# MiniMax-AI/VTP

Hardware: AMD Instinct MI355X
Metric: images/sec/node VTP-B f16d64 256x256 train step (higher is better)
Workload: dtype bf16

## Files before the change

vtp_amd/csrc/attention_resident.hip:

```cpp
#include "common.h"
#include <algorithm>
#include <cstdio>
#include <cstdlib>
#include "vtp_hip.h"

namespace vtp {

constexpr float LOG2E_R = 1.4426950408889634f;
constexpr float LN2_R = 0.6931471805599453f;
constexpr int RES_MAXN = 320;
constexpr int RES_SPLIT_COLS = 4;

struct AttnResArgs {
  const bf16 *q, *k, *v, *o, *d_o;
  bf16 *out, *dq, *dk, *dv;
  float* lse;
  float* delta;
  const bf16 *rope_sin, *rope_cos;
  int rope_prefix;
  int B, N, heads, npad;
  long sb, sn, sbo, sno;
  float scale;
  int stagger;
  long long* timing;
};

#define BWD_STAMP(i)                                                                                                     \
  do {                                                                                                                   \
    if (__builtin_expect(p.timing != nullptr, 0) && lane == 0)                                                           \
      p.timing[((((size_t)blockIdx.z * gridDim.y + blockIdx.y) * gridDim.x + blockIdx.x) * 16 + wave) * 4 + (i)] = wall_clock64(); \
  } while (0)

__device__ __forceinline__ int swz_key(int r) { return (((r >> 1) & 1) << 2) | ((r >> 2) & 3); }

__device__ __forceinline__ void stage_resident(const bf16* __restrict__ base, long sn, int N, int npad, char* lds, int wave,
                                               int nwaves, int lane) {
  const int rr = lane >> 3, cp = lane & 7;
  for (int piece = wave; piece < (npad >> 3); piece += nwaves) {
    const int row = piece * 8 + rr;
    const int c = cp ^ swz_key(row);
    const bf16* src = base + (long)min(row, N - 1) * sn + c * 8;
    __builtin_amdgcn_global_load_lds((const __attribute__((address_space(1))) void*)src,
                                     (__attribute__((address_space(3))) void*)(lds + piece * 1024), 16, 0, 0);
  }
}

__device__ __forceinline__ bf16x8 frag_row(const char* lds, int row0, int ks, int lane) {
  const int r = row0 + (lane & 31);
  return *(const bf16x8*)(lds + r * 128 + (((2 * ks + (lane >> 5)) ^ swz_key(r)) << 4));
}
__device__ __forceinline__ bf16x8 frag_tr(const char* lds, int dblk, int row0, int ks, int lane) {
  const int i = lane & 15, g = (lane >> 4) & 1, hi = lane >> 5;
  const int r = row0 + ks * 16 + hi * 4 + (i >> 2);
  const int col = dblk * 32 + g * 16 + (i & 3) * 4;
  const char* p0 = lds + r * 128 + (((col >> 3) ^ swz_key(r)) << 4) + ((col & 7) << 1);
  const char* p1 = lds + (r + 8) * 128 + (((col >> 3) ^ swz_key(r + 8)) << 4) + ((col & 7) << 1);
  bf16x4 lo = __builtin_amdgcn_ds_read_tr16_b64_v4bf16((__attribute__((address_space(3))) bf16x4*)p0);
  bf16x4 hi4 = __builtin_amdgcn_ds_read_tr16_b64_v4bf16((__attribute__((address_space(3))) bf16x4*)p1);
  return __builtin_shufflevector(lo, hi4, 0, 1, 2, 3, 4, 5, 6, 7);
}

__device__ __forceinline__ int row_part(int lane) {
  const int r = lane & 31;
  return r * 128 + (((lane >> 5) ^ swz_key(r)) << 4);
}
__device__ __forceinline__ int tr_part(int lane, int half) {
  const int i = lane & 15, g = (lane >> 4) & 1, hi = lane >> 5;
  const int r = hi * 4 + (i >> 2) + 8 * half;
  const int col = g * 16 + (i & 3) * 4;
  return r * 128 + (((col >> 3) ^ swz_key(r)) << 4) + ((col & 7) << 1);
}
__device__ __forceinline__ int lds_addr(int lane_part, int uniform_part) {
  int a;
// ... 123 lines not shown
  for (int kb = 0; kb < nkb; ++kb) {
    f32x16 s;
    zero16r(s);
#pragma unroll
    for (int ks = 0; ks < 4; ++ks) s = __builtin_amdgcn_mfma_f32_32x32x16_bf16(frag_row(Ks, kb * 32, ks, lane), qf[ks], s, 0, 0, 0);
#pragma unroll
    for (int r = 0; r < 16; ++r) s[r] = fast_exp2(s[r] * sc2 - m2);
    if (kb == last) {
#pragma unroll
      for (int r = 0; r < 16; ++r)
        if (kb * 32 + (r & 3) + 8 * (r >> 2) + 4 * hi >= p.N) s[r] = 0.f;
    }
#pragma unroll
    for (int r = 0; r < 16; ++r) l += s[r];
    const bf16x8 pf0 = pack8r(s, 0), pf1 = pack8r(s, 8);
#pragma unroll
    for (int db = 0; db < 2; ++db) {
      oacc[db] = __builtin_amdgcn_mfma_f32_32x32x16_bf16(frag_tr(Vs, db, kb * 32, 0, lane), pf0, oacc[db], 0, 0, 0);
      oacc[db] = __builtin_amdgcn_mfma_f32_32x32x16_bf16(frag_tr(Vs, db, kb * 32, 1, lane), pf1, oacc[db], 0, 0, 0);
    }
  }
  l += __shfl_xor(l, 32, 64);
  if (qi >= p.N) return;
  const float inv = 1.f / l;
  bf16* orow = p.out + (long)b * p.sbo + (long)qi * p.sno + h * 64;
#pragma unroll
  for (int db = 0; db < 2; ++db)
#pragma unroll
    for (int g = 0; g < 4; ++g) {
      f32x4 v;
#pragma unroll
      for (int e = 0; e < 4; ++e) v[e] = oacc[db][4 * g + e] * inv;
      *(bf16x4*)(orow + db * 32 + 8 * g + 4 * hi) = __builtin_convertvector(v, bf16x4);
    }
  if (hi == 0 && p.lse) p.lse[((long)b * p.heads + h) * p.N + qi] = (m2 + log2f(l)) * LN2_R;
}

__device__ __forceinline__ float both_halves_sum(float x) {
  const auto r = __builtin_amdgcn_permlane32_swap(__float_as_uint(x), __float_as_uint(x), false, false);
  return __uint_as_float(r[0]) + __uint_as_float(r[1]);
}

__device__ __forceinline__ float max3f(float a, float b, float c) {
  float r;
  asm("v_max3_f32 %0, %1, %2, %3" : "=v"(r) : "v"(a), "v"(b), "v"(c));
  return r;
}
__device__ __forceinline__ float max2f(float a, float b) {
  float r;
  asm("v_max_f32 %0, %1, %2" : "=v"(r) : "v"(a), "v"(b));
  return r;
}

constexpr float LAZY_LOG2 = 6.f;

template <int T>
__device__ __forceinline__ void attn_key_loop(const char* Ks, const char* Vs, const bf16x8 (&qf)[T][4], int N, int nkb, int kb0, int step,
                                              float sc2, int lane, f32x16 (&oacc)[T][2], float (&m)[T], float (&l)[T],
                                              int stream_ops = 0) {
  const int hi = lane >> 5, last = nkb - 1;
  const f32x16 zero = {0.f, 0.f, 0.f, 0.f, 0.f, 0.f, 0.f, 0.f, 0.f, 0.f, 0.f, 0.f, 0.f, 0.f, 0.f, 0.f};
  const f32x2 sc2v = {sc2, sc2};
#pragma unroll
  for (int t = 0; t < T; ++t) {
    oacc[t][0] = zero;
    oacc[t][1] = zero;
    m[t] = -INFINITY;
    l[t] = 0.f;
  }
  for (int kb = kb0; kb < nkb; kb += step) {
    if (stream_ops > 0 && (kb == 2 || kb == 5)) {
      wait_vmcnt_upto(__builtin_amdgcn_readfirstlane(kb == 2 ? stream_ops * max(nkb - 5, 0) : 0));
      __builtin_amdgcn_s_barrier();
      asm volatile("" ::: "memory");
    }
    f32x16 s[T];
    {
      bf16x8 kf[4];
#pragma unroll
      for (int ks = 0; ks < 4; ++ks) kf[ks] = frag_row(Ks, kb * 32, ks, lane);
#pragma unroll
      for (int t = 0; t < T; ++t) {
        s[t] = __builtin_amdgcn_mfma_f32_32x32x16_bf16(kf[0], qf[t][0], zero, 0, 0, 0);
#pragma unroll
        for (int ks = 1; ks < 4; ++ks) s[t] = __builtin_amdgcn_mfma_f32_32x32x16_bf16(kf[ks], qf[t][ks], s[t], 0, 0, 0);
      }
    }
    bf16x8 vf[2][2];
#pragma unroll
    for (int db = 0; db < 2; ++db)
#pragma unroll
      for (int ks = 0; ks < 2; ++ks) vf[db][ks] = frag_tr(Vs, db, kb * 32, ks, lane);
    if (kb == last && (N & 31)) {
#pragma unroll
      for (int t = 0; t < T; ++t)
#pragma unroll
        for (int r = 0; r < 16; ++r)
          if (kb * 32 + (r & 3) + 8 * (r >> 2) + 4 * hi >= N) s[t][r] = -INFINITY;
    }
    float mn[T];
    bool moved = false;
#pragma unroll
    for (int t = 0; t < T; ++t) {
      float bm = max3f(s[t][0], s[t][1], s[t][2]);
#pragma unroll
      for (int r = 3; r < 15; r += 2) bm = max3f(bm, s[t][r], s[t][r + 1]);
// ... 48 lines not shown
  for (int db = 0; db < 2; ++db)
#pragma unroll
    for (int j = 0; j < 2; ++j) {
      uint32_t x[2], y[2];
#pragma unroll
      for (int w = 0; w < 2; ++w) {
        const f32x2 vx = {o[db][8 * j + 2 * w] * inv, o[db][8 * j + 2 * w + 1] * inv};
        const f32x2 vy = {o[db][8 * j + 4 + 2 * w] * inv, o[db][8 * j + 4 + 2 * w + 1] * inv};
        const bf16x2 bx = __builtin_convertvector(vx, bf16x2), by = __builtin_convertvector(vy, bf16x2);
        x[w] = __builtin_bit_cast(uint32_t, bx);
        y[w] = __builtin_bit_cast(uint32_t, by);
      }
      uint32_t out[4];
#pragma unroll
      for (int w = 0; w < 2; ++w) {
        const auto r = __builtin_amdgcn_permlane32_swap(x[w], y[w], false, false);
        out[w] = r[0];
        out[2 + w] = r[1];
      }
      if (valid) {
        typedef __attribute__((ext_vector_type(4))) uint32_t u32x4;
        *(u32x4*)(orow + db * 32 + 16 * j + 8 * hi) = u32x4{out[0], out[1], out[2], out[3]};
      }
    }
}

__device__ __forceinline__ void stage_piece_asm(const bf16* base, long sn, int N, int piece, unsigned img_off, int lane) {
  const int row = piece * 8 + (lane >> 3);
  const int c = (lane & 7) ^ swz_key(row);
  const unsigned voff = (unsigned)(min(row, N - 1) * (int)sn + c * 8) * 2u;
  const unsigned dst = __builtin_amdgcn_readfirstlane(img_off + piece * 1024);
  unsigned keep;
  asm volatile("s_mov_b32 %0, m0\n\ts_mov_b32 m0, %3\n\ts_nop 0\n\tglobal_load_lds_dwordx4 %1, %2\n\ts_mov_b32 m0, %0"
               : "=&s"(keep)
               : "v"(voff), "s"(base), "s"(dst)
               : "memory");
}
__device__ __forceinline__ void stage_block_asm(const bf16* kbase, const bf16* vbase, long sn, int N, int kb, unsigned img, int wave,
                                                int nwaves, int lane) {
  for (int j = wave; j < 4; j += nwaves) {
    stage_piece_asm(kbase, sn, N, kb * 4 + j, 0, lane);
    stage_piece_asm(vbase, sn, N, kb * 4 + j, img, lane);
  }
}

#define ATTN_TSTAMP(i)                                                                            \
  do {                                                                                            \
    if (p.delta && blockIdx.x == 3 && blockIdx.y == 5 && lane == 0)                               \
      ((long long*)p.delta)[wave * 8 + (i)] = __builtin_readcyclecounter();                       \
  } while (0)

__global__ __launch_bounds__(256, 2) void attn_fwd_res2_kernel(const AttnResArgs p) {
  extern __shared__ __attribute__((aligned(16))) char smem[];
  char* Ks = smem;
  char* Vs = smem + p.npad * 128;
  float* part = (float*)(smem + 2 * p.npad * 128);
  const int lane = threadIdx.x & 63, wave = threadIdx.x >> 6, nwaves = blockDim.x >> 6, hi = lane >> 5;
  const int h = blockIdx.x, b = blockIdx.y;
  const bf16* qb = p.q + (long)b * p.sb + h * 64;
  const int ntiles = p.npad >> 5, nkb = ntiles, q0 = wave * 64;
  ATTN_TSTAMP(0);
  const bool split_last = (ntiles & 1) && ntiles > 1;
  const int qL = (ntiles - 1) * 32;
  bf16x8 qf[2][4], qfl[1][4];
#pragma unroll
  for (int t = 0; t < 2; ++t) {
    const bf16* qr = qb + (long)min(q0 + 32 * t + (lane & 31), p.N - 1) * p.sn + hi * 8;
#pragma unroll
    for (int ks = 0; ks < 4; ++ks) qf[t][ks] = *(const bf16x8*)(qr + ks * 16);
  }
  if (split_last) {
    const bf16* qr = qb + (long)min(qL + (lane & 31), p.N - 1) * p.sn + hi * 8;
#pragma unroll
    for (int ks = 0; ks < 4; ++ks) qfl[0][ks] = *(const bf16x8*)(qr + ks * 16);
  }
  const bf16* kbase = p.k + (long)b * p.sb + h * 64;
  const bf16* vbase = p.v + (long)b * p.sb + h * 64;
  const unsigned img = p.npad * 128;
  stage_block_asm(kbase, vbase, p.sn, p.N, 0, img, wave, nwaves, lane);
  if (nkb > 1) stage_block_asm(kbase, vbase, p.sn, p.N, 1, img, wave, nwaves, lane);
  __builtin_amdgcn_s_waitcnt(0x0F70);
  ATTN_TSTAMP(1);
  __builtin_amdgcn_s_barrier();
  asm volatile("" ::: "memory");
  ATTN_TSTAMP(2);
  for (int kb = 2; kb < nkb; ++kb) stage_block_asm(kbase, vbase, p.sn, p.N, kb, img, wave, nwaves, lane);
  const int stream_ops = 2 * ((4 - wave + nwaves - 1) / nwaves);
  const float sc2 = p.scale * LOG2E_R;
  const long srow0 = ((long)b * p.heads + h) * p.N;
  {
    f32x16 oacc[2][2];
    float m[2], l[2];
    const bool two = q0 + 32 < p.npad && !(split_last && q0 + 32 >= qL);
    if (two) attn_key_loop<2>(Ks, Vs, qf, p.N, nkb, 0, 1, sc2, lane, oacc, m, l, stream_ops);
    else {
      f32x16 (&o1)[1][2] = *(f32x16(*)[1][2])&oacc;
      attn_key_loop<1>(Ks, Vs, *(const bf16x8(*)[1][4])&qf, p.N, nkb, 0, 1, sc2, lane, o1, *(float(*)[1])&m, *(float(*)[1])&l,
                       stream_ops);
    }
    ATTN_TSTAMP(3);
#pragma unroll
    for (int t = 0; t < 2; ++t) {
      if (t == 1 && !two) break;
      const int qi = q0 + 32 * t + (lane & 31);
      const float lt = both_halves_sum(l[t]);
      const bool valid = qi < p.N;
      store_o_row(p.out + (long)b * p.sbo + (long)min(qi, p.N - 1) * p.sno + h * 64, oacc[t], 1.f / lt, hi, valid);
      if (valid && hi == 0 && p.lse) p.lse[srow0 + qi] = (m[t] + log2f(lt)) * LN2_R;
    }
  }
  ATTN_TSTAMP(4);
  if (!split_last) return;
  const int cols = p.N - qL;
  {
    f32x16 oacc[1][2];
    float m[1], l[1];
    attn_key_loop<1>(Ks, Vs, qfl, p.N, nkb, wave, nwaves, sc2, lane, oacc, m, l);
    const float lt = both_halves_sum(l[0]);
    if ((lane & 31) < cols) {
      float* dst = part + ((wave * cols + (lane & 31)) * 2 + hi) * 34;
      dst[0] = m[0];
      dst[1] = lt;
#pragma unroll
      for (int r = 0; r < 16; ++r) {
        dst[2 + r] = oacc[0][0][r];
        dst[18 + r] = oacc[0][1][r];
      }
    }
  }
  ATTN_TSTAMP(5);
  __syncthreads();
  ATTN_TSTAMP(6);
  if (wave != 0) return;
  {
    const int c = min(lane & 31, cols - 1);
    float M = -INFINITY;
    for (int w = 0; w < nwaves; ++w) M = fmaxf(M, part[((w * cols + c) * 2 + hi) * 34]);
    f32x16 o[2];
    zero16r(o[0]);
    zero16r(o[1]);
    float L = 0.f;
    for (int w = 0; w < nwaves; ++w) {
      const float* src = part + ((w * cols + c) * 2 + hi) * 34;
      const float sc = fast_exp2(src[0] - M);
      L += src[1] * sc;
#pragma unroll
      for (int r = 0; r < 16; ++r) {
        o[0][r] += src[2 + r] * sc;
        o[1][r] += src[18 + r] * sc;
      }
    }
    const int qi = qL + (lane & 31);
    const bool valid = (lane & 31) < cols;
    store_o_row(p.out + (long)b * p.sbo + (long)min(qi, p.N - 1) * p.sno + h * 64, o, 1.f / L, hi, valid);
    if (valid && hi == 0 && p.lse) p.lse[srow0 + qi] = (M + log2f(L)) * LN2_R;
  }
}

__global__ __launch_bounds__(640) void attn_bwd_dq_res_kernel(const AttnResArgs p) {
  extern __shared__ __attribute__((aligned(16))) char smem[];
  char* Ks = smem;
  char* Vs = smem + p.npad * 128;
  const int lane = threadIdx.x & 63, wave = threadIdx.x >> 6, nwaves = blockDim.x >> 6, hi = lane >> 5;
  const int h = blockIdx.x, b = blockIdx.y;
// ... 167 lines not shown
      for (int e2 = 0; e2 < 2; ++e2) {
        const int r = 4 * g + 2 * e2;
        f32x2 e = {s[r], s[r + 1]}, gq = {dp[r], dp[r + 1]};
        e = __builtin_elementwise_fma(e, sc2v, f32x2{l4[2 * e2], l4[2 * e2 + 1]});
        gq = __builtin_elementwise_fma(gq, scv, f32x2{d4[2 * e2], d4[2 * e2 + 1]});
        e[0] = fast_exp2(e[0]);
        e[1] = fast_exp2(e[1]);
        if (qblk == last && (p.N & 31)) {
          if (qblk * 32 + 8 * g + 4 * hi + 2 * e2 >= p.N) e[0] = 0.f;
          if (qblk * 32 + 8 * g + 4 * hi + 2 * e2 + 1 >= p.N) e[1] = 0.f;
        }
        pr[r] = e[0];
        pr[r + 1] = e[1];
        e *= gq;
        s[r] = e[0];
        s[r + 1] = e[1];
      }
    }
    const bf16x8 p0 = pack8r(pr, 0), p1 = pack8r(pr, 8), d0 = pack8r(s, 0), d1 = pack8r(s, 8);
#pragma unroll
    for (int db = 0; db < 2; ++db) {
      const int tq0 = lds_addr(tpart[db][0], q_off), tq1 = lds_addr(tpart[db][1], q_off);
      const int tg0 = lds_addr(tpart[db][0], q_off + g_off), tg1 = lds_addr(tpart[db][1], q_off + g_off);
      dv[db] = __builtin_amdgcn_mfma_f32_32x32x16_bf16(frag_tr_at(tg0, tg1, 0), p0, dv[db], 0, 0, 0);
      dv[db] = __builtin_amdgcn_mfma_f32_32x32x16_bf16(frag_tr_at(tg0, tg1, 1), p1, dv[db], 0, 0, 0);
      dk[db] = __builtin_amdgcn_mfma_f32_32x32x16_bf16(frag_tr_at(tq0, tq1, 0), d0, dk[db], 0, 0, 0);
      dk[db] = __builtin_amdgcn_mfma_f32_32x32x16_bf16(frag_tr_at(tq0, tq1, 1), d1, dk[db], 0, 0, 0);
    }
  }
  BWD_STAMP(2);
  if (ki < p.N) {
  bf16* krow = p.dk + (long)b * p.sb + (long)ki * p.sn + h * 64;
  bf16* vrow = p.dv + (long)b * p.sb + (long)ki * p.sn + h * 64;
  const bool rot = p.rope_sin && ki >= p.rope_prefix;
  const long t = (long)(ki - p.rope_prefix) * 64;
#pragma unroll
  for (int g = 0; g < 4; ++g) {
    f32x4 lo, hv, c0, c1;
#pragma unroll
    for (int e = 0; e < 4; ++e) {
      lo[e] = dk[0][4 * g + e];
      hv[e] = dk[1][4 * g + e];
      c0[e] = dv[0][4 * g + e];
      c1[e] = dv[1][4 * g + e];
    }
    store_grad_pair(krow, 8 * g + 4 * hi, lo, hv, rot ? p.rope_sin : nullptr, p.rope_cos, t);
    store_grad_pair(vrow, 8 * g + 4 * hi, c0, c1, nullptr, nullptr, 0);
  }
  }
  BWD_STAMP(3);
}

constexpr int PB_WAVES = 8;
constexpr int PB_XROWS = 2;

__device__ __forceinline__ int stage_image_asm(const bf16* base, long sn, int N, int npad, unsigned img_off, int wave, int nwaves,
                                               int lane) {
  int n = 0;
  for (int piece = wave; piece < (npad >> 3); piece += nwaves, ++n) stage_piece_asm(base, sn, N, piece, img_off, lane);
  return n;
}

__device__ __forceinline__ void dq_step(const bf16x8 (&qf)[4], const bf16x8 (&dof)[4], f32x16 (&dq)[2], const int (&rpart)[4],
                                        const int (&tpart)[2][2], int koff, int img, f32x2 sc2v, f32x2 nlse, f32x2 scv, f32x2 ndlt,
                                        int key0, int N, bool mask, int hi) {
  f32x16 s, dp;
  zero16r(s);
  zero16r(dp);
#pragma unroll
  for (int ks = 0; ks < 4; ++ks) {
    s = __builtin_amdgcn_mfma_f32_32x32x16_bf16(frag_row_at(lds_addr(rpart[ks], koff)), qf[ks], s, 0, 0, 0);
    dp = __builtin_amdgcn_mfma_f32_32x32x16_bf16(frag_row_at(lds_addr(rpart[ks], koff + img)), dof[ks], dp, 0, 0, 0);
  }
#pragma unroll
  for (int i = 0; i < 8; ++i) {
    f32x2 e = {s[2 * i], s[2 * i + 1]}, g = {dp[2 * i], dp[2 * i + 1]};
    e = __builtin_elementwise_fma(e, sc2v, nlse);
    g = __builtin_elementwise_fma(g, scv, ndlt);
    e[0] = fast_exp2(e[0]);
    e[1] = fast_exp2(e[1]);
    e *= g;
    s[2 * i] = e[0];
    s[2 * i + 1] = e[1];
  }
  if (mask) {
#pragma unroll
    for (int r = 0; r < 16; ++r)
      if (key0 + (r & 3) + 8 * (r >> 2) + 4 * hi >= N) s[r] = 0.f;
  }
  const bf16x8 d0 = pack8r(s, 0), d1 = pack8r(s, 8);
#pragma unroll
  for (int db = 0; db < 2; ++db) {
    const int t0 = lds_addr(tpart[db][0], koff), t1 = lds_addr(tpart[db][1], koff);
    dq[db] = __builtin_amdgcn_mfma_f32_32x32x16_bf16(frag_tr_at(t0, t1, 0), d0, dq[db], 0, 0, 0);
    dq[db] = __builtin_amdgcn_mfma_f32_32x32x16_bf16(frag_tr_at(t0, t1, 1), d1, dq[db], 0, 0, 0);
  }
}

__device__ __forceinline__ float row_delta(const bf16x8 (&of)[4], const bf16x8 (&dof)[4]) {
  float dlt = 0.f;
#pragma unroll
  for (int ks = 0; ks < 4; ++ks)
#pragma unroll
    for (int e = 0; e < 8; ++e) dlt += bf2f(of[ks][e]) * bf2f(dof[ks][e]);
  return dlt + __shfl_xor(dlt, 32, 64);
}

// ... 24 lines not shown
      f32x2 e = {s[r], s[r + 1]}, gq = {dp[r], dp[r + 1]};
      e = __builtin_elementwise_fma(e, sc2v, f32x2{l4[2 * e2], l4[2 * e2 + 1]});
      gq = __builtin_elementwise_fma(gq, scv, f32x2{d4[2 * e2], d4[2 * e2 + 1]});
      e[0] = fast_exp2(e[0]);
      e[1] = fast_exp2(e[1]);
      if (mask) {
        if (q0 + 8 * g + 4 * hi + 2 * e2 >= N) e[0] = 0.f;
        if (q0 + 8 * g + 4 * hi + 2 * e2 + 1 >= N) e[1] = 0.f;
      }
      pr[r] = e[0];
      pr[r + 1] = e[1];
      e *= gq;
      s[r] = e[0];
      s[r + 1] = e[1];
    }
  }
  const bf16x8 p0 = pack8r(pr, 0), p1 = pack8r(pr, 8), d0 = pack8r(s, 0), d1 = pack8r(s, 8);
#pragma unroll
  for (int db = 0; db < 2; ++db) {
    const int tq0 = lds_addr(tpart[db][0], qoff), tq1 = lds_addr(tpart[db][1], qoff);
    const int tg0 = lds_addr(tpart[db][0], qoff + img), tg1 = lds_addr(tpart[db][1], qoff + img);
    dv[db] = __builtin_amdgcn_mfma_f32_32x32x16_bf16(frag_tr_at(tg0, tg1, 0), p0, dv[db], 0, 0, 0);
    dv[db] = __builtin_amdgcn_mfma_f32_32x32x16_bf16(frag_tr_at(tg0, tg1, 1), p1, dv[db], 0, 0, 0);
    dk[db] = __builtin_amdgcn_mfma_f32_32x32x16_bf16(frag_tr_at(tq0, tq1, 0), d0, dk[db], 0, 0, 0);
    dk[db] = __builtin_amdgcn_mfma_f32_32x32x16_bf16(frag_tr_at(tq0, tq1, 1), d1, dk[db], 0, 0, 0);
  }
}

__device__ __forceinline__ void put_slot(float* slot, const f32x16 (&acc)[2], int hi) {
#pragma unroll
  for (int db = 0; db < 2; ++db)
#pragma unroll
    for (int g = 0; g < 4; ++g) {
      f32x4 v;
#pragma unroll
      for (int e = 0; e < 4; ++e) v[e] = acc[db][4 * g + e];
      *(f32x4*)(slot + 32 * db + 8 * g + 4 * hi) = v;
    }
}
__device__ __forceinline__ void store_acc_rows(bf16* row, const f32x16 (&acc)[2], int hi, const bf16* sin_t, const bf16* cos_t, long t) {
#pragma unroll
  for (int g = 0; g < 4; ++g) {
    f32x4 lo, hv;
#pragma unroll
    for (int e = 0; e < 4; ++e) {
      lo[e] = acc[0][4 * g + e];
      hv[e] = acc[1][4 * g + e];
    }
    store_grad_pair(row, 8 * g + 4 * hi, lo, hv, sin_t, cos_t, t);
  }
}

template <int W>
__global__ __launch_bounds__(64 * W) void attn_bwd_fused_kernel(const AttnResArgs p) {
  extern __shared__ __attribute__((aligned(16))) char smem[];
  const int lane = threadIdx.x & 63, wave = threadIdx.x >> 6, hi = lane >> 5;
  const int img = p.npad * 128, nb = p.npad >> 5, last = nb - 1;
  const bool odd = nb > W;
  const int nx = odd ? p.N - 32 * W : 0;
  const int QO = 0, KO = img, VO = 2 * img, GO = 3 * img;
  float* lse_s = (float*)(smem + 4 * img);
  float* dlt_s = lse_s + p.npad;
  float* xq = dlt_s + p.npad;
  float* xk = xq + (W + 1) * PB_XROWS * 64;
  float* xv = xk + (W + 1) * PB_XROWS * 64;
  const int hid = blockIdx.x, b = hid / p.heads, h = hid - b * p.heads;
  PB_STAMP(0);
  stage_image_asm(p.q + (long)b * p.sb + h * 64, p.sn, p.N, p.npad, QO, wave, W, lane);
  stage_image_asm(p.d_o + (long)b * p.sbo + h * 64, p.sno, p.N, p.npad, GO, wave, W, lane);
  stage_image_asm(p.k + (long)b * p.sb + h * 64, p.sn, p.N, p.npad, KO, wave, W, lane);
  stage_image_asm(p.v + (long)b * p.sb + h * 64, p.sn, p.N, p.npad, VO, wave, W, lane);
  const float sc2 = p.scale * LOG2E_R;
  const f32x2 sc2v = {sc2, sc2}, scv = {p.scale, p.scale};
  int rpart[4], tpart[2][2];
#pragma unroll
  for (int ks = 0; ks < 4; ++ks) rpart[ks] = row_part(lane) ^ (ks << 5);
#pragma unroll
  for (int db = 0; db < 2; ++db)
#pragma unroll
    for (int hf = 0; hf < 2; ++hf) tpart[db][hf] = tr_part(lane, hf) ^ (db << 6);
  const long srow0 = ((long)b * p.heads + h) * p.N;
  const int ri = wave * 32 + (lane & 31);
  const int rx = 32 * W + (lane & 31);
  bf16x8 of[4], of2[4];
  float lse_raw, lse_raw2 = 0.f;
  {
    const int qc = min(ri, p.N - 1);
    const bf16* orow = p.o + (long)b * p.sbo + h * 64 + (long)qc * p.sno + hi * 8;
#pragma unroll
    for (int ks = 0; ks < 4; ++ks) of[ks] = *(const bf16x8*)(orow + ks * 16);
    lse_raw = p.lse[srow0 + qc];
    if (odd) {
      const int qc2 = min(rx, p.N - 1);
      const bf16* orow2 = p.o + (long)b * p.sbo + h * 64 + (long)qc2 * p.sno + hi * 8;
#pragma unroll
      for (int ks = 0; ks < 4; ++ks) of2[ks] = *(const bf16x8*)(orow2 + ks * 16);
      lse_raw2 = p.lse[srow0 + qc2];
    }
  }
  wait_all_dma();
  __syncthreads();
  PB_STAMP(1);
  {
    bf16x8 qf[4], dof[4];
    const int own = __builtin_amdgcn_readfirstlane(wave * 4096);
#pragma unroll
    for (int ks = 0; ks < 4; ++ks) {
// ... 75 lines not shown
      zero16r(dv[1]);
      for (int qb = 0; qb < nb; ++qb)
        dkv_step(kf, vf, dk, dv, rpart, tpart, __builtin_amdgcn_readfirstlane(QO + qb * 4096), GO - QO, lse_s, dlt_s, sc2v, scv, qb * 32,
                 p.N, qb == last && (p.N & 31), hi);
      if (ri < p.N) {
        const bool rot = p.rope_sin && ri >= p.rope_prefix;
        store_acc_rows(p.dk + (long)b * p.sb + (long)ri * p.sn + h * 64, dk, hi, rot ? p.rope_sin : nullptr, p.rope_cos,
                       (long)(ri - p.rope_prefix) * 64);
        store_acc_rows(p.dv + (long)b * p.sb + (long)ri * p.sn + h * 64, dv, hi, nullptr, nullptr, 0);
      }
    }
    if (odd) {
      const int ox = __builtin_amdgcn_readfirstlane(W * 4096);
#pragma unroll
      for (int ks = 0; ks < 4; ++ks) {
        kf[ks] = frag_row_at(lds_addr(rpart[ks], KO + ox));
        vf[ks] = frag_row_at(lds_addr(rpart[ks], VO + ox));
      }
      for (int qb = wave; qb < nb; qb += W) {
        f32x16 dkx[2], dvx[2];
        zero16r(dkx[0]);
        zero16r(dkx[1]);
        zero16r(dvx[0]);
        zero16r(dvx[1]);
        dkv_step(kf, vf, dkx, dvx, rpart, tpart, __builtin_amdgcn_readfirstlane(QO + qb * 4096), GO - QO, lse_s, dlt_s, sc2v, scv,
                 qb * 32, p.N, qb == last && (p.N & 31), hi);
        if ((lane & 31) < nx) {
          put_slot(xk + (qb * PB_XROWS + (lane & 31)) * 64, dkx, hi);
          put_slot(xv + (qb * PB_XROWS + (lane & 31)) * 64, dvx, hi);
        }
      }
    }
  }
  if (odd) {
    __syncthreads();
    if ((int)threadIdx.x < nx * 8) {
      const int row = threadIdx.x >> 3, d0 = 4 * (threadIdx.x & 7), krow_i = 32 * W + row;
      f32x4 lo = {0.f, 0.f, 0.f, 0.f}, hv = lo, c0 = lo, c1 = lo;
      for (int qb = 0; qb < nb; ++qb) {
        lo += *(const f32x4*)(xk + (qb * PB_XROWS + row) * 64 + d0);
        hv += *(const f32x4*)(xk + (qb * PB_XROWS + row) * 64 + 32 + d0);
        c0 += *(const f32x4*)(xv + (qb * PB_XROWS + row) * 64 + d0);
        c1 += *(const f32x4*)(xv + (qb * PB_XROWS + row) * 64 + 32 + d0);
      }
      const bool rot = p.rope_sin && krow_i >= p.rope_prefix;
      store_grad_pair(p.dk + (long)b * p.sb + (long)krow_i * p.sn + h * 64, d0, lo, hv, rot ? p.rope_sin : nullptr, p.rope_cos,
                      (long)(krow_i - p.rope_prefix) * 64);
      store_grad_pair(p.dv + (long)b * p.sb + (long)krow_i * p.sn + h * 64, d0, c0, c1, nullptr, nullptr, 0);
    }
  }
  PB_STAMP(3);
}

static int res_waves_per_block(int nw, int groups) {
  return (groups <= 512 && nw >= 4) ? (nw + 1) / 2 : nw;
}

template <typename K>
static void set_lds(K kern, int bytes) {
  hipFuncSetAttribute((const void*)kern, hipFuncAttributeMaxDynamicSharedMemorySize, bytes);
}

static long long* g_attn_timing = nullptr;
static int g_attn_wpb = 0;
static int g_attn_lds_pad = 0;
static int g_attn_stagger = 0;

int attn_resident_fwd(const void* q, const void* k, const void* v, void* o, float* lse, int B, int N, int heads, long sb,
                      long sn, long sbo, long sno, float scale, hipStream_t s) {
  AttnResArgs a = {};
  a.q = (const bf16*)q; a.k = (const bf16*)k; a.v = (const bf16*)v; a.out = (bf16*)o; a.lse = lse;
  a.B = B; a.N = N; a.heads = heads; a.npad = (N + 31) / 32 * 32; a.sb = sb; a.sn = sn; a.sbo = sbo; a.sno = sno; a.scale = scale;
  static bool attr = false;
  if (!attr) {
    set_lds(attn_fwd_res_kernel, 2 * RES_MAXN * 128);
    set_lds(attn_fwd_res2_kernel, 2 * RES_MAXN * 128 + 5 * RES_SPLIT_COLS * 2 * 34 * 4);
    attr = true;
  }
  {
    const int ntiles = a.npad / 32, cols = N - 32 * (ntiles - 1);
    const bool odd = (ntiles & 1) && ntiles > 1;
    if (!odd || cols <= RES_SPLIT_COLS) {
      const int waves = std::max(1, ntiles / 2);
      const int lds = 2 * a.npad * 128 + (odd ? waves * cols * 2 * 34 * 4 : 0);
      static long long* tbuf = nullptr;
      static const bool timing = getenv("VTP_ATTN_TIMING") != nullptr;
      if (timing && !tbuf && hipMalloc((void**)&tbuf, 64 * 8) != hipSuccess) tbuf = nullptr;
      if (timing) a.delta = (float*)tbuf;
      hipLaunchKernelGGL(attn_fwd_res2_kernel, dim3(heads, B), dim3(64 * waves), lds, s, a);
      if (timing && tbuf) {
        int occ = -1;
        (void)hipOccupancyMaxActiveBlocksPerMultiprocessor(&occ, attn_fwd_res2_kernel, 64 * waves, lds);
        fprintf(stderr, "[attn timing] workgroups per CU by the runtime's count: %d (lds %d B, %d waves)\n", occ, lds, waves);
        long long hbuf[64];
        (void)hipStreamSynchronize(s);
        (void)hipMemcpy(hbuf, tbuf, sizeof hbuf, hipMemcpyDeviceToHost);
        for (int w = 0; w < waves; ++w) {
          fprintf(stderr, "[attn timing] wave %d:", w);
          for (int i = 1; i < 7; ++i) fprintf(stderr, " t%d=%lld", i, hbuf[w * 8 + i] - hbuf[0]);
          fprintf(stderr, "\n");
        }
      }
      return check_launch("attn_fwd_resident2");
    }
  }
  const int nw = a.npad / 32, wpb = res_waves_per_block(nw, heads * B);
  hipLaunchKernelGGL(attn_fwd_res_kernel, dim3(heads, B, (nw + wpb - 1) / wpb), dim3(64 * wpb), 2 * a.npad * 128, s, a);
  return check_launch("attn_fwd_resident");
}

int attn_resident_bwd(const void* q, const void* k, const void* v, const void* o, const void* d_o, const float* lse,
                      float* delta, void* dq, void* dk, void* dv, const void* rope_sin, const void* rope_cos, int rope_prefix,
                      int B, int N, int heads, long sb, long sn, long sbo, long sno, float scale, hipStream_t s) {
  AttnResArgs a = {};
  a.q = (const bf16*)q; a.k = (const bf16*)k; a.v = (const bf16*)v; a.o = (const bf16*)o; a.d_o = (const bf16*)d_o;
  a.lse = (float*)lse; a.delta = delta; a.dq = (bf16*)dq; a.dk = (bf16*)dk; a.dv = (bf16*)dv;
  a.rope_sin = (const bf16*)rope_sin; a.rope_cos = (const bf16*)rope_cos; a.rope_prefix = rope_prefix;
  a.B = B; a.N = N; a.heads = heads; a.npad = (N + 31) / 32 * 32; a.sb = sb; a.sn = sn; a.sbo = sbo; a.sno = sno; a.scale = scale;
  a.timing = g_attn_timing;
  a.stagger = g_attn_stagger;
  static bool attr = false;
  if (!attr) {
    set_lds(attn_bwd_dq_res_kernel, 2 * RES_MAXN * 128 + 32768);
    set_lds(attn_bwd_dkv_res_kernel, 2 * RES_MAXN * 128 + 8 * RES_MAXN + 32768);
    attr = true;
  }
  const int nw = a.npad / 32;
  auto fits = [&](int W) { return nw == W || (nw == W + 1 && N - 32 * W <= PB_XROWS); };
  const bool off32 = (long)N * sn * 2 < (1L << 31) && (long)N * sno * 2 < (1L << 31);
  if (g_attn_wpb == 0 && off32 && (fits(PB_WAVES) || fits(2))) {
    auto lds_of = [](int npad, int W) { return 4 * npad * 128 + 8 * npad + 3 * (W + 1) * PB_XROWS * 256; };
    static bool attr_p = false;
    if (!attr_p) {
      set_lds(attn_bwd_fused_kernel<PB_WAVES>, lds_of(32 * (PB_WAVES + 1), PB_WAVES));
      set_lds(attn_bwd_fused_kernel<2>, lds_of(32 * 3, 2));
      attr_p = true;
    }
    if (fits(PB_WAVES))
      hipLaunchKernelGGL(attn_bwd_fused_kernel<PB_WAVES>, dim3(B * heads), dim3(64 * PB_WAVES), lds_of(a.npad, PB_WAVES), s, a);
    else
      hipLaunchKernelGGL(attn_bwd_fused_kernel<2>, dim3(B * heads), dim3(128), lds_of(a.npad, 2), s, a);
    return check_launch("attn_bwd_fused");
  }
  const int wpb = g_attn_wpb > 0 ? std::min(g_attn_wpb, nw) : res_waves_per_block(nw, heads * B);
  const dim3 grid(heads, B, (nw + wpb - 1) / wpb), block(64 * wpb);
  if (a.timing) {
    int o1 = -1, o2 = -1;
    (void)hipOccupancyMaxActiveBlocksPerMultiprocessor(&o1, attn_bwd_dq_res_kernel, block.x, 2 * a.npad * 128);
    (void)hipOccupancyMaxActiveBlocksPerMultiprocessor(&o2, attn_bwd_dkv_res_kernel, block.x, 2 * a.npad * 128 + 8 * a.npad);
    fprintf(stderr, "[attn timing] workgroups per CU by the runtime's count: dQ %d, dK/dV %d (%d waves, lds %d / %d B)\n", o1, o2,
            (int)block.x / 64, 2 * a.npad * 128, 2 * a.npad * 128 + 8 * a.npad);
  }
  hipLaunchKernelGGL(attn_bwd_dq_res_kernel, grid, block, 2 * a.npad * 128 + g_attn_lds_pad, s, a);
  if (a.timing) a.timing += (size_t)grid.x * grid.y * grid.z * 64;
  hipLaunchKernelGGL(attn_bwd_dkv_res_kernel, grid, block, 2 * a.npad * 128 + 8 * a.npad + g_attn_lds_pad, s, a);
  return check_launch("attn_bwd_resident");
}

}

extern "C" int vtp_attn_debug(void* timing, int lds_pad, int waves_per_wg, int stagger_ticks) {
  vtp::g_attn_stagger = stagger_ticks;
  vtp::g_attn_wpb = waves_per_wg;
  vtp::g_attn_timing = (long long*)timing;
  vtp::g_attn_lds_pad = lds_pad;
  return 0;
}
```

Measured before the change: 741.8.

## Handle few extra tokens as side rows instead of padding a full 32-row tile

```diff
diff --git a/vtp_amd/csrc/attention_resident.hip b/vtp_amd/csrc/attention_resident.hip
--- a/vtp_amd/csrc/attention_resident.hip
+++ b/vtp_amd/csrc/attention_resident.hip
@@ -10,6 +10,7 @@
 constexpr float LN2_R = 0.6931471805599453f;
 constexpr int RES_MAXN = 320;
 constexpr int RES_SPLIT_COLS = 4;
+constexpr int PB_XROWS = 2;
 
 struct AttnResArgs {
   const bf16 *q, *k, *v, *o, *d_o;
@@ -19,6 +20,7 @@
   const bf16 *rope_sin, *rope_cos;
   int rope_prefix;
   int B, N, heads, npad;
+  int xrows;
   long sb, sn, sbo, sno;
   float scale;
   int stagger;
@@ -248,6 +250,47 @@
   return r;
 }
 
+__device__ __forceinline__ const char* img_chunk(const char* img, int r, int c) { return img + r * 128 + ((c ^ swz_key(r)) << 4); }
+
+__device__ __forceinline__ float dot_frag_row(const bf16x8 (&f)[4], const char* img, int r, int hi) {
+  float acc = 0.f;
+#pragma unroll
+  for (int ks = 0; ks < 4; ++ks) {
+    const bf16x8 x = *(const bf16x8*)img_chunk(img, r, 2 * ks + hi);
+#pragma unroll
+    for (int j = 0; j < 4; ++j)
+      acc = __builtin_amdgcn_fdot2_f32_bf16(bf16x2{f[ks][2 * j], f[ks][2 * j + 1]}, bf16x2{x[2 * j], x[2 * j + 1]}, acc, false);
+  }
+  return both_halves_sum(acc);
+}
+
+__device__ __forceinline__ void axpy_acc(f32x16 (&acc)[2], float w, const char* img, int r, int hi) {
+#pragma unroll
+  for (int db = 0; db < 2; ++db)
+#pragma unroll
+    for (int g = 0; g < 4; ++g) {
+      const bf16x4 x = *(const bf16x4*)(img_chunk(img, r, 4 * db + g) + 8 * hi);
+#pragma unroll
+      for (int e = 0; e < 4; ++e) acc[db][4 * g + e] = fmaf(w, bf2f(x[e]), acc[db][4 * g + e]);
+    }
+}
+
+__device__ __forceinline__ f32x2 wsum_rows32(const char* img, int r0, const float* w, int lane) {
+  const int dp = lane & 31, hi = lane >> 5;
+  f32x2 acc = {0.f, 0.f};
+#pragma unroll
+  for (int j4 = 0; j4 < 4; ++j4) {
+    const f32x4 w4 = *(const f32x4*)(w + 16 * hi + 4 * j4);
+#pragma unroll
+    for (int e = 0; e < 4; ++e) {
+      const bf16x2 x = *(const bf16x2*)(img_chunk(img, r0 + 16 * hi + 4 * j4 + e, dp >> 2) + (dp & 3) * 4);
+      acc[0] = fmaf(w4[e], bf2f(x[0]), acc[0]);
+      acc[1] = fmaf(w4[e], bf2f(x[1]), acc[1]);
+    }
+  }
+  return f32x2{both_halves_sum(acc[0]), both_halves_sum(acc[1])};
+}
+
 constexpr float LAZY_LOG2 = 6.f;
 
 template <int T>
@@ -402,13 +445,16 @@
 
 __global__ __launch_bounds__(256, 2) void attn_fwd_res2_kernel(const AttnResArgs p) {
   extern __shared__ __attribute__((aligned(16))) char smem[];
+  const int xr = p.xrows;
+  const unsigned img = (p.npad + (xr ? 8 : 0)) * 128;
   char* Ks = smem;
-  char* Vs = smem + p.npad * 128;
-  float* part = (float*)(smem + 2 * p.npad * 128);
+  char* Vs = smem + img;
+  float* part = (float*)(smem + 2 * img);
   const int lane = threadIdx.x & 63, wave = threadIdx.x >> 6, nwaves = blockDim.x >> 6, hi = lane >> 5;
   const int h = blockIdx.x, b = blockIdx.y;
   const bf16* qb = p.q + (long)b * p.sb + h * 64;
   const int ntiles = p.npad >> 5, nkb = ntiles, q0 = wave * 64;
+  const int Nm = p.N - xr;
   ATTN_TSTAMP(0);
   const bool split_last = (ntiles & 1) && ntiles > 1;
   const int qL = (ntiles - 1) * 32;
@@ -426,9 +472,16 @@
   }
   const bf16* kbase = p.k + (long)b * p.sb + h * 64;
   const bf16* vbase = p.v + (long)b * p.sb + h * 64;
-  const unsigned img = p.npad * 128;
   stage_block_asm(kbase, vbase, p.sn, p.N, 0, img, wave, nwaves, lane);
   if (nkb > 1) stage_block_asm(kbase, vbase, p.sn, p.N, 1, img, wave, nwaves, lane);
+  if (xr) {
+    const int pc = 4 * nkb;
+    if (wave == 0) {
+      stage_piece_asm(kbase, p.sn, p.N, pc, 0, lane);
+      stage_piece_asm(vbase, p.sn, p.N, pc, img, lane);
+    }
+    if (wave == nwaves - 1) stage_piece_asm(qb, p.sn, p.N, pc, 2 * img - pc * 1024, lane);
+  }
   __builtin_amdgcn_s_waitcnt(0x0F70);
   ATTN_TSTAMP(1);
   __builtin_amdgcn_s_barrier();
@@ -442,11 +495,40 @@
     f32x16 oacc[2][2];
     float m[2], l[2];
     const bool two = q0 + 32 < p.npad && !(split_last && q0 + 32 >= qL);
-    if (two) attn_key_loop<2>(Ks, Vs, qf, p.N, nkb, 0, 1, sc2, lane, oacc, m, l, stream_ops);
+    if (two) attn_key_loop<2>(Ks, Vs, qf, Nm, nkb, 0, 1, sc2, lane, oacc, m, l, stream_ops);
     else {
       f32x16 (&o1)[1][2] = *(f32x16(*)[1][2])&oacc;
-      attn_key_loop<1>(Ks, Vs, *(const bf16x8(*)[1][4])&qf, p.N, nkb, 0, 1, sc2, lane, o1, *(float(*)[1])&m, *(float(*)[1])&l,
+      attn_key_loop<1>(Ks, Vs, *(const bf16x8(*)[1][4])&qf, Nm, nkb, 0, 1, sc2, lane, o1, *(float(*)[1])&m, *(float(*)[1])&l,
                        stream_ops);
+    }
+    if (xr) {
+      for (int x = 0; x < xr; ++x) {
+        const int rk = p.npad + x;
+        float cand[2];
+        bool moved = false;
+#pragma unroll
+        for (int t = 0; t < 2; ++t) {
+          cand[t] = dot_frag_row(qf[t], Ks, rk, hi) * sc2;
+          moved |= cand[t] > m[t] + LAZY_LOG2;
+        }
+        if (__any(moved)) {
+#pragma unroll
+          for (int t = 0; t < 2; ++t) {
+            const float mn = cand[t] > m[t] + LAZY_LOG2 ? cand[t] : m[t];
+            const float alpha = fast_exp2(m[t] - mn);
+            l[t] *= alpha;
+            oacc[t][0] *= alpha;
+            oacc[t][1] *= alpha;
+            m[t] = mn;
+          }
+        }
+#pragma unroll
+        for (int t = 0; t < 2; ++t) {
+          const float pv = fast_exp2(cand[t] - m[t]);
+          if (hi == 0) l[t] += pv;
+          axpy_acc(oacc[t], pv, Vs, rk, hi);
+        }
+      }
     }
     ATTN_TSTAMP(3);
 #pragma unroll
@@ -460,6 +542,77 @@
     }
   }
   ATTN_TSTAMP(4);
+  if (xr) {
+    const char* Qx = smem + 2 * img - p.npad * 128;
+    float* pw = part + 256;
+    float* pm = pw + nwaves * PB_XROWS * 68;
+    const int k = 64 * wave + lane;
+    const bool xkey = wave == nwaves - 1 && lane < xr;
+    const int k2 = p.npad + min(lane, xr - 1);
+    float s[PB_XROWS], s2[PB_XROWS];
+#pragma unroll
+    for (int x = 0; x < PB_XROWS; ++x) s[x] = s2[x] = 0.f;
+#pragma unroll
+    for (int c = 0; c < 8; ++c) {
+      const bf16x8 kc = *(const bf16x8*)img_chunk(Ks, k, c);
+      const bf16x8 kc2 = *(const bf16x8*)img_chunk(Ks, k2, c);
+#pragma unroll
+      for (int x = 0; x < PB_XROWS; ++x) {
+        if (x >= xr) break;
+        const bf16x8 qc = *(const bf16x8*)img_chunk(Qx, p.npad + x, c);
+#pragma unroll
+        for (int j = 0; j < 4; ++j) {
+          const bf16x2 qv = {qc[2 * j], qc[2 * j + 1]};
+          s[x] = __builtin_amdgcn_fdot2_f32_bf16(bf16x2{kc[2 * j], kc[2 * j + 1]}, qv, s[x], false);
+          s2[x] = __builtin_amdgcn_fdot2_f32_bf16(bf16x2{kc2[2 * j], kc2[2 * j + 1]}, qv, s2[x], false);
+        }
+      }
+    }
+#pragma unroll
+    for (int x = 0; x < PB_XROWS; ++x) {
+      if (x >= xr) break;
+      float* px = pw + (wave * PB_XROWS + x) * 68;
+      const float mw = wave_max(xkey ? fmaxf(s[x], s2[x]) : s[x]) * sc2;
+      const float p1 = fast_exp2(s[x] * sc2 - mw), p2 = xkey ? fast_exp2(s2[x] * sc2 - mw) : 0.f;
+      const float lw = wave_sum(p1 + p2);
+      px[lane] = p1;
+      if (xkey) px[64 + lane] = p2;
+      __builtin_amdgcn_wave_barrier();
+      asm volatile("" ::: "memory");
+      f32x2 o = wsum_rows32(Vs, 64 * wave, px, lane) + wsum_rows32(Vs, 64 * wave + 32, px + 32, lane);
+      if (wave == nwaves - 1)
+        for (int y = 0; y < xr; ++y) {
+          const bf16x2 v2 = *(const bf16x2*)(img_chunk(Vs, p.npad + y, (lane & 31) >> 2) + (lane & 3) * 4);
+          o[0] = fmaf(px[64 + y], bf2f(v2[0]), o[0]);
+          o[1] = fmaf(px[64 + y], bf2f(v2[1]), o[1]);
+        }
+      float* dst = pm + (wave * PB_XROWS + x) * 68;
+      if (lane == 0) {
+        dst[0] = mw;
+        dst[1] = lw;
+      }
+      if (hi == 0) *(f32x2*)(dst + 4 + 2 * lane) = o;
+    }
+    ATTN_TSTAMP(5);
+    __syncthreads();
+    ATTN_TSTAMP(6);
+    if (wave != 0 || hi >= xr) return;
+    const int x = hi, dp = lane & 31;
+    float M = -INFINITY, L = 0.f;
+    for (int w = 0; w < nwaves; ++w) M = fmaxf(M, pm[(w * PB_XROWS + x) * 68]);
+    f32x2 o = {0.f, 0.f};
+    for (int w = 0; w < nwaves; ++w) {
+      const float* src = pm + (w * PB_XROWS + x) * 68;
+      const float sc = fast_exp2(src[0] - M);
+      L += src[1] * sc;
+      o += *(const f32x2*)(src + 4 + 2 * dp) * sc;
+    }
+    const float inv = 1.f / L;
+    const long qx = p.npad + x;
+    *(bf16x2*)(p.out + (long)b * p.sbo + qx * p.sno + h * 64 + 2 * dp) = __builtin_convertvector(o * inv, bf16x2);
+    if (dp == 0 && p.lse) p.lse[srow0 + qx] = (M + log2f(L)) * LN2_R;
+    return;
+  }
   if (!split_last) return;
   const int cols = p.N - qL;
   {
@@ -733,7 +886,6 @@
 }
 
 constexpr int PB_WAVES = 8;
-constexpr int PB_XROWS = 2;
 
 __device__ __forceinline__ int stage_image_asm(const bf16* base, long sn, int N, int npad, unsigned img_off, int wave, int nwaves,
                                                int lane) {
@@ -864,7 +1016,7 @@
 }
 
 template <int W>
-__global__ __launch_bounds__(64 * W) void attn_bwd_fused_kernel(const AttnResArgs p) {
+__global__ __launch_bounds__(64 * W) void attn_bwd_fused_pad_kernel(const AttnResArgs p) {
   extern __shared__ __attribute__((aligned(16))) char smem[];
   const int lane = threadIdx.x & 63, wave = threadIdx.x >> 6, hi = lane >> 5;
   const int img = p.npad * 128, nb = p.npad >> 5, last = nb - 1;
@@ -1046,6 +1198,216 @@
   PB_STAMP(3);
 }
 
+template <int W>
+__global__ __launch_bounds__(64 * W) void attn_bwd_fused_kernel(const AttnResArgs p) {
+  extern __shared__ __attribute__((aligned(16))) char smem[];
+  const int lane = threadIdx.x & 63, wave = threadIdx.x >> 6, hi = lane >> 5;
+  constexpr int NM = 32 * W;
+  const int xr = max(p.N - NM, 0);
+  const int rows = NM + (xr ? 8 : 0);
+  const int img = rows * 128, last = W - 1;
+  const bool mask_last = p.N < NM && (p.N & 31);
+  const int QO = 0, KO = img, VO = 2 * img, GO = 3 * img;
+  float* lse_s = (float*)(smem + 4 * img);
+  float* dlt_s = lse_s + rows;
+  float* wq = dlt_s + rows;
+  float* wk = wq + 2 * PB_XROWS * NM;
+  float* xpart = wk + PB_XROWS * NM;
+  float* xc = xpart + W * 3 * PB_XROWS * 64;
+  const char *Qi = smem + QO, *Ki = smem + KO, *Vi = smem + VO, *Gi = smem + GO;
+  const int hid = blockIdx.x, b = hid / p.heads, h = hid - b * p.heads;
+  PB_STAMP(0);
+  stage_image_asm(p.q + (long)b * p.sb + h * 64, p.sn, p.N, rows, QO, wave, W, lane);
+  stage_image_asm(p.d_o + (long)b * p.sbo + h * 64, p.sno, p.N, rows, GO, wave, W, lane);
+  stage_image_asm(p.k + (long)b * p.sb + h * 64, p.sn, p.N, rows, KO, wave, W, lane);
+  stage_image_asm(p.v + (long)b * p.sb + h * 64, p.sn, p.N, rows, VO, wave, W, lane);
+  const float sc2 = p.scale * LOG2E_R;
+  const f32x2 sc2v = {sc2, sc2}, scv = {p.scale, p.scale};
+  int rpart[4], tpart[2][2];
+#pragma unroll
+  for (int ks = 0; ks < 4; ++ks) rpart[ks] = row_part(lane) ^ (ks << 5);
+#pragma unroll
+  for (int db = 0; db < 2; ++db)
+#pragma unroll
+    for (int hf = 0; hf < 2; ++hf) tpart[db][hf] = tr_part(lane, hf) ^ (db << 6);
+  const long srow0 = ((long)b * p.heads + h) * p.N;
+  const int ri = wave * 32 + (lane & 31);
+  const bool xwave = xr && wave == W - 1;
+  const int rx = NM + min(lane & 31, max(xr, 1) - 1);
+  bf16x8 of[4], of2[4];
+  float lse_raw, lse_raw2 = 0.f;
+  {
+    const int qc = min(ri, p.N - 1);
+    const bf16* orow = p.o + (long)b * p.sbo + h * 64 + (long)qc * p.sno + hi * 8;
+#pragma unroll
+    for (int ks = 0; ks < 4; ++ks) of[ks] = *(const bf16x8*)(orow + ks * 16);
+    lse_raw = p.lse[srow0 + qc];
+    if (xwave) {
+      const bf16* orow2 = p.o + (long)b * p.sbo + h * 64 + (long)rx * p.sno + hi * 8;
+#pragma unroll
+      for (int ks = 0; ks < 4; ++ks) of2[ks] = *(const bf16x8*)(orow2 + ks * 16);
+      lse_raw2 = p.lse[srow0 + rx];
+    }
+  }
+  wait_all_dma();
+  __syncthreads();
+  PB_STAMP(1);
+  {
+    bf16x8 qf[4], dof[4];
+    const int own = __builtin_amdgcn_readfirstlane(wave * 4096);
+#pragma unroll
+    for (int ks = 0; ks < 4; ++ks) {
+      qf[ks] = frag_row_at(lds_addr(rpart[ks], QO + own));
+      dof[ks] = frag_row_at(lds_addr(rpart[ks], GO + own));
+    }
+    const float dlt = row_delta(of, dof);
+    if (hi == 0) {
+      lse_s[ri] = -lse_raw * LOG2E_R;
+      dlt_s[ri] = -dlt * p.scale;
+      if (ri < p.N) p.delta[srow0 + ri] = dlt;
+    }
+    const float lse2 = lse_raw * LOG2E_R;
+    {
+      const f32x2 nlse = {-lse2, -lse2}, ndlt = {-dlt * p.scale, -dlt * p.scale};
+      f32x16 dq[2];
+      zero16r(dq[0]);
+      zero16r(dq[1]);
+      for (int kb = 0; kb < W; ++kb)
+        dq_step(qf, dof, dq, rpart, tpart, __builtin_amdgcn_readfirstlane(KO + kb * 4096), img, sc2v, nlse, scv, ndlt, kb * 32, p.N,
+                kb == last && mask_last, hi);
+#pragma unroll
+      for (int x = 0; x < PB_XROWS; ++x) {
+        if (x >= xr) break;
+        const float sv = dot_frag_row(qf, Ki, NM + x, hi), dpv = dot_frag_row(dof, Vi, NM + x, hi);
+        const float pv = fast_exp2(fmaf(sv, sc2, -lse2));
+        const float ds = pv * fmaf(dpv, p.scale, -dlt * p.scale);
+        axpy_acc(dq, ds, Ki, NM + x, hi);
+        if (hi == 0) {
+          wq[x * NM + ri] = pv;
+          wq[(PB_XROWS + x) * NM + ri] = ds;
+        }
+      }
+      if (ri < p.N) {
+        const bool rot = p.rope_sin && ri >= p.rope_prefix;
+        store_acc_rows(p.dq + (long)b * p.sb + (long)ri * p.sn + h * 64, dq, hi, rot ? p.rope_sin : nullptr, p.rope_cos,
+                       (long)(ri - p.rope_prefix) * 64);
+      }
+    }
+    if (xr) {
+      __builtin_amdgcn_wave_barrier();
+      asm volatile("" ::: "memory");
+#pragma unroll
+      for (int x = 0; x < PB_XROWS; ++x) {
+        if (x >= xr) break;
+        const f32x2 dkp = wsum_rows32(Qi, wave * 32, wq + (PB_XROWS + x) * NM + wave * 32, lane);
+        const f32x2 dvp = wsum_rows32(Gi, wave * 32, wq + x * NM + wave * 32, lane);
+        if (hi == 0) {
+          *(f32x2*)(xpart + ((wave * 3 + 0) * PB_XROWS + x) * 64 + 2 * lane) = dkp;
+          *(f32x2*)(xpart + ((wave * 3 + 1) * PB_XROWS + x) * 64 + 2 * lane) = dvp;
+        }
+      }
+    }
+    if (xwave) {
+      bf16x8 qx[4], dox[4];
+#pragma unroll
+      for (int ks = 0; ks < 4; ++ks) {
+        qx[ks] = *(const bf16x8*)img_chunk(Qi, rx, 2 * ks + hi);
+        dox[ks] = *(const bf16x8*)img_chunk(Gi, rx, 2 * ks + hi);
+      }
+      const float dlt2 = row_delta(of2, dox), lse2x = lse_raw2 * LOG2E_R;
+      const bool own_x = hi == 0 && (lane & 31) < xr;
+      if (own_x) {
+        lse_s[rx] = -lse2x;
+        dlt_s[rx] = -dlt2 * p.scale;
+        p.delta[srow0 + rx] = dlt2;
+      }
+#pragma unroll
+      for (int y = 0; y < PB_XROWS; ++y) {
+        if (y >= xr) break;
+        const float sv = dot_frag_row(qx, Ki, NM + y, hi), dpv = dot_frag_row(dox, Vi, NM + y, hi);
+        const float pv = fast_exp2(fmaf(sv, sc2, -lse2x));
+        const float ds = pv * fmaf(dpv, p.scale, -dlt2 * p.scale);
+        if (own_x) {
+          xc[(lane & 31) * PB_XROWS + y] = pv;
+          xc[(PB_XROWS + (lane & 31)) * PB_XROWS + y] = ds;
+        }
+      }
+    }
+  }
+  __syncthreads();
+  PB_STAMP(2);
+  {
+    bf16x8 kf[4], vf[4];
+    const int own = __builtin_amdgcn_readfirstlane(wave * 4096);
+#pragma unroll
+    for (int ks = 0; ks < 4; ++ks) {
+      kf[ks] = frag_row_at(lds_addr(rpart[ks], KO + own));
+      vf[ks] = frag_row_at(lds_addr(rpart[ks], VO + own));
+    }
+    f32x16 dk[2], dv[2];
+    zero16r(dk[0]);
+    zero16r(dk[1]);
+    zero16r(dv[0]);
+    zero16r(dv[1]);
+    for (int qb = 0; qb < W; ++qb)
+      dkv_step(kf, vf, dk, dv, rpart, tpart, __builtin_amdgcn_readfirstlane(QO + qb * 4096), GO - QO, lse_s, dlt_s, sc2v, scv, qb * 32,
+               p.N, qb == last && mask_last, hi);
+#pragma unroll
+    for (int x = 0; x < PB_XROWS; ++x) {
+      if (x >= xr) break;
+      const float sv = dot_frag_row(kf, Qi, NM + x, hi), dpv = dot_frag_row(vf, Gi, NM + x, hi);
+      const float pv = fast_exp2(fmaf(sv, sc2, lse_s[NM + x]));
+      const float ds = pv * fmaf(dpv, p.scale, dlt_s[NM + x]);
+      axpy_acc(dv, pv, Gi, NM + x, hi);
+      axpy_acc(dk, ds, Qi, NM + x, hi);
+      if (hi == 0) wk[x * NM + ri] = ds;
+    }
+    if (ri < p.N) {
+      const bool rot = p.rope_sin && ri >= p.rope_prefix;
+      store_acc_rows(p.dk + (long)b * p.sb + (long)ri * p.sn + h * 64, dk, hi, rot ? p.rope_sin : nullptr, p.rope_cos,
+                     (long)(ri - p.rope_prefix) * 64);
+      store_acc_rows(p.dv + (long)b * p.sb + (long)ri * p.sn + h * 64, dv, hi, nullptr, nullptr, 0);
+    }
+    if (xr) {
+      __builtin_amdgcn_wave_barrier();
+      asm volatile("" ::: "memory");
+#pragma unroll
+      for (int x = 0; x < PB_XROWS; ++x) {
+        if (x >= xr) break;
+        const f32x2 dqp = wsum_rows32(Ki, wave * 32, wk + x * NM + wave * 32, lane);
+        if (hi == 0) *(f32x2*)(xpart + ((wave * 3 + 2) * PB_XROWS + x) * 64 + 2 * lane) = dqp;
+      }
+    }
+  }
+  if (xr) {
+    __syncthreads();
+    if ((int)threadIdx.x < 3 * xr * 8) {
+      const int task = threadIdx.x / (xr * 8), x = (threadIdx.x >> 3) % xr, d0 = 4 * (threadIdx.x & 7), row = NM + x;
+      f32x4 lo = {0.f, 0.f, 0.f, 0.f}, hv = lo;
+      for (int w = 0; w < W; ++w) {
+        const float* src = xpart + ((w * 3 + task) * PB_XROWS + x) * 64;
+        lo += *(const f32x4*)(src + d0);
+        hv += *(const f32x4*)(src + 32 + d0);
+      }
+      const char* cimg = task == 0 ? Qi : task == 1 ? Gi : Ki;
+      for (int y = 0; y < xr; ++y) {
+        const float c = task == 0 ? xc[(PB_XROWS + y) * PB_XROWS + x] : task == 1 ? xc[y * PB_XROWS + x] : xc[(PB_XROWS + x) * PB_XROWS + y];
+        const bf16x4 a4 = *(const bf16x4*)(img_chunk(cimg, NM + y, d0 >> 3) + (d0 & 7) * 2);
+        const bf16x4 b4 = *(const bf16x4*)(img_chunk(cimg, NM + y, (d0 + 32) >> 3) + (d0 & 7) * 2);
+#pragma unroll
+        for (int e = 0; e < 4; ++e) {
+          lo[e] = fmaf(c, bf2f(a4[e]), lo[e]);
+          hv[e] = fmaf(c, bf2f(b4[e]), hv[e]);
+        }
+      }
+      bf16* dst = (task == 0 ? p.dk : task == 1 ? p.dv : p.dq) + (long)b * p.sb + (long)row * p.sn + h * 64;
+      const bool rot = task != 1 && p.rope_sin && row >= p.rope_prefix;
+      store_grad_pair(dst, d0, lo, hv, rot ? p.rope_sin : nullptr, p.rope_cos, (long)(row - p.rope_prefix) * 64);
+    }
+  }
+  PB_STAMP(3);
+}
+
 static int res_waves_per_block(int nw, int groups) {
   return (groups <= 512 && nw >= 4) ? (nw + 1) / 2 : nw;
 }
@@ -1059,6 +1421,14 @@
 static int g_attn_wpb = 0;
 static int g_attn_lds_pad = 0;
 static int g_attn_stagger = 0;
+
+static bool attn_padded() {
+  static const bool env = [] {
+    const char* e = getenv("VTP_ATTN_PADDED");
+    return e != nullptr && atoi(e) != 0;
+  }();
+  return env || g_attn_wpb == -2;
+}
 
 int attn_resident_fwd(const void* q, const void* k, const void* v, void* o, float* lse, int B, int N, int heads, long sb,
                       long sn, long sbo, long sno, float scale, hipStream_t s) {
@@ -1071,12 +1441,17 @@
     set_lds(attn_fwd_res2_kernel, 2 * RES_MAXN * 128 + 5 * RES_SPLIT_COLS * 2 * 34 * 4);
     attr = true;
   }
+  if (N > 32 && (N & 31) <= PB_XROWS && ((N >> 5) & 1) == 0 && !attn_padded()) {
+    a.xrows = N & 31;
+    a.npad = N - a.xrows;
+  }
   {
     const int ntiles = a.npad / 32, cols = N - 32 * (ntiles - 1);
     const bool odd = (ntiles & 1) && ntiles > 1;
     if (!odd || cols <= RES_SPLIT_COLS) {
       const int waves = std::max(1, ntiles / 2);
-      const int lds = 2 * a.npad * 128 + (odd ? waves * cols * 2 * 34 * 4 : 0);
+      const int lds = a.xrows ? 2 * (a.npad + 8) * 128 + 1024 + 2 * waves * PB_XROWS * 68 * 4
+                              : 2 * a.npad * 128 + (odd ? waves * cols * 2 * 34 * 4 : 0);
       static long long* tbuf = nullptr;
       static const bool timing = getenv("VTP_ATTN_TIMING") != nullptr;
       if (timing && !tbuf && hipMalloc((void**)&tbuf, 64 * 8) != hipSuccess) tbuf = nullptr;
@@ -1122,18 +1497,32 @@
   const int nw = a.npad / 32;
   auto fits = [&](int W) { return nw == W || (nw == W + 1 && N - 32 * W <= PB_XROWS); };
   const bool off32 = (long)N * sn * 2 < (1L << 31) && (long)N * sno * 2 < (1L << 31);
-  if (g_attn_wpb == 0 && off32 && (fits(PB_WAVES) || fits(2))) {
-    auto lds_of = [](int npad, int W) { return 4 * npad * 128 + 8 * npad + 3 * (W + 1) * PB_XROWS * 256; };
+  if ((g_attn_wpb == 0 || g_attn_wpb == -2) && off32 && (fits(PB_WAVES) || fits(2))) {
+    auto lds_pad = [](int npad, int W) { return 4 * npad * 128 + 8 * npad + 3 * (W + 1) * PB_XROWS * 256; };
+    auto lds_sb = [](int N, int W) {
+      const int rows = 32 * W + (N > 32 * W ? 8 : 0);
+      return 4 * rows * 128 + 8 * rows +
+             (N > 32 * W ? 4 * (3 * PB_XROWS * 32 * W + W * 3 * PB_XROWS * 64 + 2 * PB_XROWS * PB_XROWS) : 0);
+    };
     static bool attr_p = false;
     if (!attr_p) {
-      set_lds(attn_bwd_fused_kernel<PB_WAVES>, lds_of(32 * (PB_WAVES + 1), PB_WAVES));
-      set_lds(attn_bwd_fused_kernel<2>, lds_of(32 * 3, 2));
+      set_lds(attn_bwd_fused_kernel<PB_WAVES>, lds_sb(32 * PB_WAVES + PB_XROWS, PB_WAVES));
+      set_lds(attn_bwd_fused_kernel<2>, lds_sb(64 + PB_XROWS, 2));
+      set_lds(attn_bwd_fused_pad_kernel<PB_WAVES>, lds_pad(32 * (PB_WAVES + 1), PB_WAVES));
+      set_lds(attn_bwd_fused_pad_kernel<2>, lds_pad(32 * 3, 2));
       attr_p = true;
     }
-    if (fits(PB_WAVES))
-      hipLaunchKernelGGL(attn_bwd_fused_kernel<PB_WAVES>, dim3(B * heads), dim3(64 * PB_WAVES), lds_of(a.npad, PB_WAVES), s, a);
-    else
-      hipLaunchKernelGGL(attn_bwd_fused_kernel<2>, dim3(B * heads), dim3(128), lds_of(a.npad, 2), s, a);
+    const int W = fits(PB_WAVES) ? PB_WAVES : 2;
+    if (nw > W && attn_padded()) {
+      if (W == PB_WAVES)
+        hipLaunchKernelGGL(attn_bwd_fused_pad_kernel<PB_WAVES>, dim3(B * heads), dim3(64 * W), lds_pad(a.npad, W), s, a);
+      else
+        hipLaunchKernelGGL(attn_bwd_fused_pad_kernel<2>, dim3(B * heads), dim3(64 * W), lds_pad(a.npad, W), s, a);
+    } else if (W == PB_WAVES) {
+      hipLaunchKernelGGL(attn_bwd_fused_kernel<PB_WAVES>, dim3(B * heads), dim3(64 * W), lds_sb(N, W), s, a);
+    } else {
+      hipLaunchKernelGGL(attn_bwd_fused_kernel<2>, dim3(B * heads), dim3(64 * W), lds_sb(N, W), s, a);
+    }
     return check_launch("attn_bwd_fused");
   }
   const int wpb = g_attn_wpb > 0 ? std::min(g_attn_wpb, nw) : res_waves_per_block(nw, heads * B);
```

Result: no change. 743.7, median of 6 (+0.3%).
